# learningOrchestra/learningOrchestra

Measured on NVIDIA H100. Metric: rows/sec project+cast+histogram 100M×32 fp64→fp32; HBM GB/s vs peak @1/2/4/8 GPU, higher is better.
Workload: dtype f64->f32

## Files before the change

### learningorchestra_b200/csrc/kernels.cuh

```cuda
#pragma once
#include <cstdint>
#include <cuda_runtime.h>
#include "parse_number.cuh"
#include "format_number.cuh"

namespace lo {

constexpr int kThreads      = 256;
constexpr int kVec          = 4;
constexpr int kBatch        = 4;
constexpr int kBatches      = 15;
constexpr int kVecPerThread = kBatch * kBatches;
constexpr int kElemsPerThread = kVec * kVecPerThread;
constexpr int kTileRows     = kThreads * kElemsPerThread;
constexpr int kHalf         = kThreads * kVec / 2;
constexpr int kHistRows     = 64;
constexpr int kHistSmemBytes = (kHistRows * kThreads + 256) * 4;

#ifndef LO_PF_BATCH
#define LO_PF_BATCH 5
#endif
#ifndef LO_PF_NBUF
#define LO_PF_NBUF 2
#endif
// ... 295 lines not shown
    __threadfence();
    asm volatile("red.release.gpu.global.add.u64 [%0], %1;" :: "l"(G.gen), "l"(1ull) : "memory");
    asm volatile("st.release.gpu.global.u64 [%0], %1;" :: "l"(G.epi_seq), "l"(G.step + 1ull) : "memory");
}

__device__ __forceinline__ void group_root_epilogue(const GroupStep &G, int n, int first, int stride, bool signal) {
    for (int i = first; i < n; i += stride) {
        const unsigned long long c = ld_relaxed_sys(G.shared + i);
        G.result[i] = c;
        for (int p = 0; p < G.npeers; ++p)
            if (G.peer_result[p]) G.peer_result[p][i] = c;
        G.shared[i] = 0ull;
    }
    if (signal) {
        __syncthreads();
        __threadfence_system();
        if ((int)threadIdx.x < G.npeers) red_release_sys_add(G.peer_clean[threadIdx.x], 1ull);
    }
}

__device__ __forceinline__ void group_wait_generation(const GroupStep &G) {
    if (G.gen_target == 0ull) return;
    if (threadIdx.x == 0) {
        unsigned long long v;
        const unsigned long long t0 = globaltimer_ns();
        for (;;) {
            asm volatile("ld.acquire.gpu.global.u64 %0, [%1];" : "=l"(v) : "l"(G.gen) : "memory");
            if (v >= G.gen_target) break;
            if (globaltimer_ns() - t0 > G.timeout_ns) { atomicAdd(G.timed_out, 1ull); break; }
            __nanosleep(64);
        }
    }
    __syncthreads();
}

__device__ __forceinline__ void group_finish_column(const GroupStep &G, unsigned j, int nb, int k, unsigned tiles_per_col,
                                                    volatile uint32_t *sflag) {
    __syncthreads();
    if (threadIdx.x == 0) {
        __threadfence();
        *sflag = (atomicAdd(G.col_ticket + j, 1u) == tiles_per_col - 1u) ? 1u : 0u;
    }
    __syncthreads();
    if (*sflag == 0u) return;
    __threadfence();
    if (threadIdx.x == 0) {
        G.col_ticket[j] = 0u;
        if (G.clean) wait_flag_ge(G.clean, G.clean_target, G.timeout_ns, G.timed_out);
    }
    __syncthreads();
    for (int b = threadIdx.x; b < nb; b += blockDim.x) {
        unsigned long long *src = G.local + (long long)j * nb + b;
        const unsigned long long c = ld_relaxed_gpu(src);
        if (c) {
            asm volatile("red.relaxed.sys.global.add.u64 [%0], %1;" :: "l"(G.shared + (long long)j * nb + b), "l"(c) : "memory");
            *src = 0ull;
        }
    }
    __syncthreads();
    if (threadIdx.x == 0) {
        __threadfence_system();
        const bool last = atomicAdd(G.done_ticket, 1u) == (unsigned)k - 1u;
        if (last) {
            *G.done_ticket = 0u;
            __threadfence_system();
            red_release_sys_add(G.arrived, 1ull);
            if (!G.is_root) asm volatile("red.release.gpu.global.add.u64 [%0], %1;" :: "l"(G.gen), "l"(1ull) : "memory");
        }
        *sflag = (last && G.is_root) ? 2u : 0u;
        if (*sflag == 2u) {
            epilogue_turn_wait(G);
            if (!wait_flag_ge(G.arrived, G.arrive_target, G.timeout_ns, G.timed_out)) *sflag = 3u;
        }
    }
    __syncthreads();
    if (*sflag == 2u) group_root_epilogue(G, k * nb, threadIdx.x, blockDim.x, true);
    else if (*sflag == 3u && (int)threadIdx.x < G.npeers) red_release_sys_add(G.peer_clean[threadIdx.x], 1ull);
    if (*sflag >= 2u) {
        __syncthreads();
        if (threadIdx.x == 0) epilogue_turn_done(G);
    }
}

template <int OUT, bool HIST, bool ALIGNED, bool EDGES>
__global__ void __launch_bounds__(kThreads, LO_MIN_CTAS)
k_project_cast_hist(const char *__restrict__ in_base, long long in_pitch,
                    char *__restrict__ out_base, long long out_pitch,
                    long long nrows, unsigned tiles_per_col, unsigned long long *__restrict__ counts,
                    const float *__restrict__ edges, const __grid_constant__ ColsF64 P, const __grid_constant__ GroupStep G) {
    extern __shared__ uint32_t smem[];
    if (G.overlap) asm volatile("griddepcontrol.launch_dependents;" ::: "memory");
    const unsigned j    = blockIdx.x / tiles_per_col;
    const unsigned tile = blockIdx.x - j * tiles_per_col;
    const long long r0  = (long long)tile * kTileRows;
    const long long n   = min((long long)kTileRows, nrows - r0);

    const double *in = reinterpret_cast<const double *>(in_base + (long long)P.col[j] * in_pitch) + r0;
    float  *out32 = nullptr;
    double *out64 = nullptr;
    if (OUT == 1) out32 = reinterpret_cast<float *>(out_base + (long long)j * out_pitch) + r0;
    if (OUT == 2) out64 = reinterpret_cast<double *>(out_base + (long long)j * out_pitch) + r0;

    BinParams B = {0.f, 0.f, 1.f, 1.f, 0};
    int rows = 0;
    uint8_t *priv = reinterpret_cast<uint8_t *>(smem) + 4 * threadIdx.x;
    if (HIST) {
        B.lo = P.lo[j]; B.hi = P.hi[j]; B.w = P.w[j];
        B.r = __frcp_rn(B.w);
        B.last = P.nbins - 1;
        rows = (P.nbins + 3) >> 2;
    }
    EdgeParams E = {0.f, 0.f, 0u};
    if (HIST && EDGES) {
        uint4 *tab = reinterpret_cast<uint4 *>(reinterpret_cast<char *>(smem) + kHistSmemBytes);
        load_edge_table(tab, edges + (long long)j * (P.nbins + 1), P.nbins);
        E = edge_params(B.lo, B.w, tab);
    }

    if (ALIGNED && n == kTileRows) {
        double v[kPfBuf][kPfBatch][4];
        const double *src = in + 2 * (long long)threadIdx.x;
#pragma unroll
        for (int pb = 0; pb < kPfBuf - 1; ++pb)
#pragma unroll
            for (int u = 0; u < kPfBatch; ++u)
                ldg_split4_stream(src + (long long)(pb * kPfBatch + u) * kThreads * kVec, kHalf, v[pb][u]);
        if (HIST) zero_private(smem, rows);
        const long long t2 = 2 * (long long)threadIdx.x;
#pragma unroll 1
        for (int b0 = 0; b0 < kPfBatches; b0 += kPfBuf) {
            const double *rsrc = src + (long long)b0 * (kPfBatch * kThreads * kVec);
            float  *rout32 = (OUT == 1) ? out32 + t2 + (long long)b0 * (kPfBatch * kThreads * kVec) : nullptr;
            double *rout64 = (OUT == 2) ? out64 + t2 + (long long)b0 * (kPfBatch * kThreads * kVec) : nullptr;
#pragma unroll
            for (int s = 0; s < kPfBuf; ++s) {
                const int b  = b0 + s;
                const int nb = b + kPfBuf - 1;
                if (nb < kPfBatches) {
#pragma unroll
                    for (int u = 0; u < kPfBatch; ++u)
                        ldg_split4_stream(rsrc + ((s + kPfBuf - 1) * kPfBatch + u) * kThreads * kVec, kHalf,
                                          v[(s + kPfBuf - 1) % kPfBuf][u]);
                }
#pragma unroll
                for (int u = 0; u < kPfBatch; ++u) {
                    const int e = (s * kPfBatch + u) * kThreads * kVec;
                    float f0 = cast_f64_f32(v[s][u][0]), f1 = cast_f64_f32(v[s][u][1]);
                    float f2 = cast_f64_f32(v[s][u][2]), f3 = cast_f64_f32(v[s][u][3]);
                    if (OUT == 1) stg_split4_stream(rout32 + e, kHalf, f0, f1, f2, f3);
                    if (OUT == 2) stg_split4_stream(rout64 + e, kHalf, v[s][u]);
                    if (HIST && EDGES) {
                        bump_edge(priv, f0, E); bump_edge(priv, f1, E); bump_edge(priv, f2, E); bump_edge(priv, f3, E);
                    } else if (HIST) {
                        bump4(priv, bin_index_f32<false>(f0, B), bin_index_f32<false>(f1, B),
                              bin_index_f32<false>(f2, B), bin_index_f32<false>(f3, B));
                    }
                }
            }
        }
    } else if (ALIGNED) {
        if (HIST) zero_private(smem, rows);
#pragma unroll 1
        for (int b = 0; b < kBatches; ++b) {
            const long long e0 = (long long)b * kBatch * kThreads * kVec + 2 * threadIdx.x;
            if (e0 >= n) break;
            double v[kBatch][4];
            if (e0 + (long long)(kBatch - 1) * kThreads * kVec + kHalf + 2 <= n) {
#pragma unroll
                for (int u = 0; u < kBatch; ++u) ldg_split4_stream(in + e0 + (long long)u * kThreads * kVec, kHalf, v[u]);
#pragma unroll
                for (int u = 0; u < kBatch; ++u) {
                    const long long e = e0 + (long long)u * kThreads * kVec;
                    float f0 = cast_f64_f32(v[u][0]), f1 = cast_f64_f32(v[u][1]);
                    float f2 = cast_f64_f32(v[u][2]), f3 = cast_f64_f32(v[u][3]);
                    if (OUT == 1) stg_split4_stream(out32 + e, kHalf, f0, f1, f2, f3);
                    if (OUT == 2) stg_split4_stream(out64 + e, kHalf, v[u]);
                    if (HIST && EDGES) {
                        bump_edge(priv, f0, E); bump_edge(priv, f1, E); bump_edge(priv, f2, E); bump_edge(priv, f3, E);
                    } else if (HIST) {
                        bump4(priv, bin_index_f32<false>(f0, B), bin_index_f32<false>(f1, B),
                              bin_index_f32<false>(f2, B), bin_index_f32<false>(f3, B));
                    }
                }
            } else {
#pragma unroll 1
                for (int u = 0; u < kBatch; ++u) {
                    const long long e = e0 + (long long)u * kThreads * kVec;
#pragma unroll 1
                    for (int q = 0; q < kVec; ++q) {
                        const long long eq = e + (q & 1) + (q >> 1) * kHalf;
                        if (eq < n) {
                            double x = ldg64_stream(in + eq);
                            float  f = cast_f64_f32(x);
                            if (OUT == 1) out32[eq] = f;
                            if (OUT == 2) out64[eq] = x;
                            if (HIST && EDGES) bump_edge(priv, f, E);
                            else if (HIST) bin_f32<false>(priv, f, B);
                        }
                    }
                }
            }
        }
    } else {
        if (HIST) zero_private(smem, rows);
#pragma unroll 1
        for (int i = 0; i < kElemsPerThread; ++i) {
            const long long e = (long long)i * kThreads + threadIdx.x;
            if (e >= n) break;
            double x = ldg64_stream(in + e);
            float  f = cast_f64_f32(x);
            if (OUT == 1) out32[e] = f;
            if (OUT == 2) out64[e] = x;
            if (HIST && EDGES) bump_edge(priv, f, E);
            else if (HIST) bin_f32<false>(priv, f, B);
        }
    }

    if (HIST) {
        if (G.mode == 0) {
            fold_and_flush(smem, rows, P.nbins, counts + (long long)j * P.nbins);
        } else {
            group_wait_generation(G);
            fold_and_flush(smem, rows, P.nbins, G.local + (long long)j * P.nbins);
            group_finish_column(G, j, P.nbins, P.k, tiles_per_col, smem);
        }
    }
}

constexpr int kWBThreads   = 512;
constexpr int kWBSmemWords = 16384;
constexpr int kWBSmemWordsMax = 57344;
constexpr int kWBVecs      = 4;
constexpr int kWBRoundRows = kWBThreads * kVec * kWBVecs;
// ... 705 lines not shown
```

### learningorchestra_b200/csrc/loexec.cu

```cuda
#include "loexec.h"
#include "kernels.cuh"

#include <cub/device/device_scan.cuh>

#include <algorithm>
#include <atomic>
#include <condition_variable>
#include <cctype>
#include <chrono>
#include <cmath>
#include <cstdarg>
#include <cstdio>
#include <cstdlib>
#include <cstring>
#include <memory>
#include <mutex>
#include <new>
#include <string>
#include <type_traits>
#include <utility>
#include <vector>

namespace {

thread_local std::string g_err;

int fail(int code, const char *fmt, ...) {
    char buf[512];
    va_list ap;
    va_start(ap, fmt);
    vsnprintf(buf, sizeof buf, fmt, ap);
    va_end(ap);
    g_err = buf;
    (void)cudaGetLastError();
    return code;
}

#define LO_CUDA(call)                                                                        \
    do {                                                                                     \
        cudaError_t e_ = (call);                                                             \
        if (e_ != cudaSuccess) {                                                             \
            int code_ = (e_ == cudaErrorMemoryAllocation) ? LO_ERR_NOMEM : LO_ERR_CUDA;      \
            return fail(code_, "%s failed: %s (%s:%d)", #call, cudaGetErrorString(e_),       \
                        __FILE__, __LINE__);                                                 \
        }                                                                                    \
    } while (0)

#define LO_TRY(call)                 \
    do {                             \
        int rc_ = (call);            \
        if (rc_ != LO_OK) return rc_; \
    } while (0)

size_t dtype_size(int dtype) {
    switch (dtype) {
        case LO_F64: return 8;
        case LO_F32: return 4;
        case LO_U8:  return 1;
        case LO_U32: return 4;
        default:     return 0;
    }
}

}

struct lo_table {
    int       dtype;
    int64_t   nrows;
    int32_t   ncols;
    int64_t   pitch;
    char     *base;
    bool      owned;
    int       device;
};

constexpr int kSlots = 3;
constexpr int kMaxStageSets = 4;

struct StageSet {
    cudaStream_t compute = nullptr, h2d = nullptr, d2h = nullptr;
    char        *in[kSlots]  = {nullptr, nullptr, nullptr};
    char        *out[kSlots] = {nullptr, nullptr, nullptr};
    size_t       in_bytes = 0, out_bytes = 0;
    unsigned long long *counts = nullptr;
    size_t       counts_n = 0;
    cudaEvent_t  ev_h2d[kSlots] = {}, ev_k[kSlots] = {}, ev_d2h[kSlots] = {};
};

struct EdgeTable {
    int32_t            nbins = 0;
    std::vector<float> lo, hi;
    float             *dev = nullptr;
    size_t             bytes = 0;
    cudaEvent_t        ready = nullptr;
    std::vector<cudaEvent_t> uses;
    uint64_t           last_use = 0;
};
constexpr int kEdgeTables = 8;

struct lo_ctx {
    int          device;
    int          sm_count;
    size_t       hbm_bytes;
    cudaStream_t stream;
    std::atomic<int64_t> launches{0};
    std::atomic<bool> use_tma{false};
    std::mutex   pool_mu;
    std::condition_variable pool_cv;
    std::vector<StageSet *> free_sets;
    int          nsets = 0;
    std::mutex   edge_mu;
    cudaStream_t edge_stream = nullptr;
    std::vector<std::unique_ptr<EdgeTable>> edge_tables;
    uint64_t     edge_tick = 0;
    std::atomic<int64_t> divide_launches{0};
};

namespace {

cudaStream_t pick(lo_ctx *ctx, void *stream) { return stream ? (cudaStream_t)stream : ctx->stream; }

int check_ctx(const lo_ctx *ctx) {
    if (!ctx) return fail(LO_ERR_INVALID, "ctx is NULL");
    cudaError_t e = cudaSetDevice(ctx->device);
    if (e != cudaSuccess) return fail(LO_ERR_CUDA, "cudaSetDevice(%d): %s", ctx->device, cudaGetErrorString(e));
    return LO_OK;
}

cudaError_t launched(lo_ctx *ctx, int n) {
    const cudaError_t e = cudaGetLastError();
    if (e == cudaSuccess) ctx->launches.fetch_add(n, std::memory_order_relaxed);
    return e;
}

bool aligned32(const lo_table *t) {
    return ((uintptr_t)t->base % 32 == 0) && (t->pitch % 32 == 0);
}

int check_cols(const lo_table *in, const int32_t *col_idx, int32_t k) {
    if (k <= 0) return fail(LO_ERR_INVALID, "k must be > 0 (got %d)", k);
    if (!col_idx) return fail(LO_ERR_INVALID, "col_idx is NULL");
    for (int j = 0; j < k; ++j)
        if (col_idx[j] < 0 || col_idx[j] >= in->ncols)
            return fail(LO_ERR_INVALID, "col_idx[%d] = %d outside [0, %d)", j, col_idx[j], in->ncols);
    return LO_OK;
}

int check_spec(const lo_hist_spec *spec, int32_t k, float *w_out ) {
    if (spec->nbins < 1 || spec->nbins > LO_MAX_BINS)
        return fail(LO_ERR_INVALID, "nbins = %d outside [1, %d]", spec->nbins, LO_MAX_BINS);
    if (spec->flags != 0) return fail(LO_ERR_INVALID, "unknown lo_hist_spec.flags 0x%x", spec->flags);
    if (!spec->lo || !spec->hi) return fail(LO_ERR_INVALID, "lo_hist_spec.lo / .hi is NULL");
    for (int j = 0; j < k; ++j) {
        const float lo = spec->lo[j], hi = spec->hi[j];
        volatile float span = hi - lo;
        volatile float w    = span / (float)spec->nbins;
        if (!(std::isfinite(lo) && std::isfinite(hi)) || !(hi > lo) || !std::isfinite(w) || !(w > 0.0f))
            return fail(LO_ERR_INVALID, "histogram range of column %d is not usable: lo=%g hi=%g nbins=%d",
                        j, (double)lo, (double)hi, spec->nbins);
        w_out[j] = w;
    }
    return LO_OK;
}

template <typename K>
int allow_smem(K kernel, int bytes) {
    LO_CUDA(cudaFuncSetAttribute(kernel, cudaFuncAttributeMaxDynamicSharedMemorySize, bytes));
    return LO_OK;
}

template <int OUT>
int allow_smem_hist() {
    LO_TRY(allow_smem(lo::k_project_cast_hist<OUT, true, true, true>, lo::kEdgeSmemBytes));
    LO_TRY(allow_smem(lo::k_project_cast_hist<OUT, true, true, false>, lo::kHistSmemBytes));
    LO_TRY(allow_smem(lo::k_project_cast_hist<OUT, true, false, true>, lo::kEdgeSmemBytes));
    LO_TRY(allow_smem(lo::k_project_cast_hist<OUT, true, false, false>, lo::kHistSmemBytes));
    return LO_OK;
}

bool fastdiv_ok(float w) {
    uint32_t bits;
    memcpy(&bits, &w, 4);
    if ((bits & 0x007FFFFFu) == 0x007FFFFFu) return false;
    return w >= 0x1p-100f && w <= 0x1p100f;
}

bool edges_ok(float w) { return w >= 0x1p-100f && w <= 0x1p100f; }

int bin_ieee_host(float f, float lo, float w, int last) {
// ... 91 lines not shown
        nt->bytes = n * 4;
        std::vector<float> h(n);
        for (int j = 0; j < P.k; ++j) hist_edges(P.lo[j], P.hi[j], P.w[j], P.nbins, h.data() + (size_t)j * (P.nbins + 1));
        cudaError_t e = cudaMallocAsync((void **)&nt->dev, nt->bytes, ctx->edge_stream);
        if (e == cudaSuccess) e = cudaMemcpyAsync(nt->dev, h.data(), nt->bytes, cudaMemcpyHostToDevice, ctx->edge_stream);
        if (e == cudaSuccess) e = cudaEventCreateWithFlags(&nt->ready, cudaEventDisableTiming);
        if (e == cudaSuccess) e = cudaEventRecord(nt->ready, ctx->edge_stream);
        if (e != cudaSuccess) {
            edge_retire(ctx, nt.get());
            return fail(e == cudaErrorMemoryAllocation ? LO_ERR_NOMEM : LO_ERR_CUDA, "edge table upload: %s",
                        cudaGetErrorString(e));
        }
        t = nt.get();
        ctx->edge_tables.push_back(std::move(nt));
    }
    LO_CUDA(cudaStreamWaitEvent(s, t->ready, 0));
    t->last_use = ++ctx->edge_tick;
    *out = t;
    return LO_OK;
}

int edge_used(EdgeTable *t, cudaStream_t s) {
    t->uses.erase(std::remove_if(t->uses.begin(), t->uses.end(), [](cudaEvent_t e) {
                      if (cudaEventQuery(e) != cudaSuccess) return false;
                      cudaEventDestroy(e);
                      return true;
                  }), t->uses.end());
    (void)cudaGetLastError();
    cudaEvent_t e = nullptr;
    LO_CUDA(cudaEventCreateWithFlags(&e, cudaEventDisableTiming));
    const cudaError_t r = cudaEventRecord(e, s);
    if (r != cudaSuccess) {
        cudaEventDestroy(e);
        return fail(LO_ERR_CUDA, "edge table use: %s", cudaGetErrorString(r));
    }
    t->uses.push_back(e);
    return LO_OK;
}

template <typename K>
int allow_smem_tma(K kernel) {
    LO_CUDA(cudaFuncSetAttribute(kernel, cudaFuncAttributeMaxDynamicSharedMemorySize, lo::kTmaSmemBytes));
    return LO_OK;
}

int configure_kernels() {
    LO_TRY(allow_smem_tma(lo::k_project_cast_hist_tma<0, true, true>));
    LO_TRY(allow_smem_tma(lo::k_project_cast_hist_tma<1, true, true>));
    LO_TRY(allow_smem_tma(lo::k_project_cast_hist_tma<2, true, true>));
    LO_TRY(allow_smem_tma(lo::k_project_cast_hist_tma<1, false, false>));
    LO_TRY(allow_smem_tma(lo::k_project_cast_hist_tma<2, false, false>));
    LO_TRY(allow_smem_hist<0>());
    LO_TRY(allow_smem_hist<1>());
    LO_TRY(allow_smem_hist<2>());
    LO_CUDA(cudaFuncSetAttribute(lo::k_hist_u8_cols_lanes<true>, cudaFuncAttributeMaxDynamicSharedMemorySize, lo::kU8LSmemBytes));
    LO_CUDA(cudaFuncSetAttribute(lo::k_hist_u8_cols_lanes<false>, cudaFuncAttributeMaxDynamicSharedMemorySize, lo::kU8LSmemBytes));
    LO_CUDA(cudaFuncSetAttribute(lo::k_project_cast_hist_bins<0, true>, cudaFuncAttributeMaxDynamicSharedMemorySize, lo::kWBSmemWordsMax * 4));
    LO_CUDA(cudaFuncSetAttribute(lo::k_project_cast_hist_bins<1, true>, cudaFuncAttributeMaxDynamicSharedMemorySize, lo::kWBSmemWordsMax * 4));
    LO_CUDA(cudaFuncSetAttribute(lo::k_project_cast_hist_bins<2, true>, cudaFuncAttributeMaxDynamicSharedMemorySize, lo::kWBSmemWordsMax * 4));
    LO_CUDA(cudaFuncSetAttribute(lo::k_project_cast_hist_bins<0, false>, cudaFuncAttributeMaxDynamicSharedMemorySize, lo::kWBSmemWordsMax * 4));
    LO_CUDA(cudaFuncSetAttribute(lo::k_project_cast_hist_bins<1, false>, cudaFuncAttributeMaxDynamicSharedMemorySize, lo::kWBSmemWordsMax * 4));
    LO_CUDA(cudaFuncSetAttribute(lo::k_project_cast_hist_bins<2, false>, cudaFuncAttributeMaxDynamicSharedMemorySize, lo::kWBSmemWordsMax * 4));
    return LO_OK;
}

const lo::GroupStep kNoGroup = {};

template <typename... KArgs, typename... Args>
cudaError_t launch_kernel(void (*kernel)(KArgs...), unsigned grid, unsigned block, size_t smem, cudaStream_t s, bool overlap,
                          Args &&...args) {
    cudaLaunchConfig_t cfg = {};
    cfg.gridDim = dim3(grid);
    cfg.blockDim = dim3(block);
    cfg.dynamicSmemBytes = smem;
    cfg.stream = s;
    cudaLaunchAttribute attr[1];
    attr[0].id = cudaLaunchAttributeProgrammaticStreamSerialization;
    attr[0].val.programmaticStreamSerializationAllowed = 1;
    cfg.attrs = attr;
    cfg.numAttrs = overlap ? 1 : 0;
    return cudaLaunchKernelEx(&cfg, kernel, std::forward<Args>(args)...);
}

template <int OUT, bool HIST>
int launch_f64(lo_ctx *ctx, const lo_table *in, const lo_table *out, int32_t out_col0,
               const lo::ColsF64 &P, unsigned long long *counts, bool aligned, const lo::GroupStep &G, cudaStream_t s) {
    std::unique_lock<std::mutex> edge_lock(ctx->edge_mu, std::defer_lock);
    EdgeTable *et = nullptr;
    if (HIST) {
        edge_lock.lock();
        LO_TRY(edge_acquire(ctx, P, s, &et));
        if (!et) {
            edge_lock.unlock();
            ctx->divide_launches.fetch_add(1, std::memory_order_relaxed);
        }
    }
    const float *edges = et ? et->dev : nullptr;
    const size_t smem = !HIST ? 0 : edges ? lo::kEdgeSmemBytes : lo::kHistSmemBytes;
    char *out_base = out ? out->base + (int64_t)out_col0 * out->pitch : nullptr;
    const long long out_pitch = out ? out->pitch : 0;
    bool fast = HIST;
    for (int j = 0; HIST && j < P.k; ++j) fast = fast && fastdiv_ok(P.w[j]);
    if (ctx->use_tma.load(std::memory_order_relaxed) && aligned && fast == HIST && in->nrows >= lo::kTileRows && G.mode == 0) {
        const unsigned full_tiles = (unsigned)(in->nrows / lo::kTileRows);
        const unsigned long long tblocks = (unsigned long long)full_tiles * (unsigned)P.k;
        if (tblocks > 0x7fffffffull) return fail(LO_ERR_INVALID, "table too large for one launch (%llu tiles)", tblocks);
        lo::k_project_cast_hist_tma<OUT, HIST, HIST><<<(unsigned)tblocks, lo::kThreads + 32, lo::kTmaSmemBytes, s>>>(
            in->base, in->pitch, out_base, out_pitch, in->nrows, full_tiles, counts, P);
        LO_CUDA(launched(ctx, 1));
        const int64_t done = (int64_t)full_tiles * lo::kTileRows;
        if (done == in->nrows) return LO_OK;
        const char *ib = in->base + done * 8;
        char *ob = out ? out->base + done * (int64_t)dtype_size(out->dtype) + (int64_t)out_col0 * out->pitch : nullptr;
        if (edges) lo::k_project_cast_hist<OUT, HIST, true, true><<<(unsigned)P.k, lo::kThreads, smem, s>>>(
                       ib, in->pitch, ob, out_pitch, in->nrows - done, 1u, counts, edges, P, kNoGroup);
        else       lo::k_project_cast_hist<OUT, HIST, true, false><<<(unsigned)P.k, lo::kThreads, smem, s>>>(
                       ib, in->pitch, ob, out_pitch, in->nrows - done, 1u, counts, edges, P, kNoGroup);
        LO_CUDA(launched(ctx, 1));
        if (et) LO_TRY(edge_used(et, s));
        return LO_OK;
    }
    const unsigned tiles_per_col = (unsigned)((in->nrows + lo::kTileRows - 1) / lo::kTileRows);
    const unsigned long long blocks = (unsigned long long)tiles_per_col * (unsigned)P.k;
    if (blocks > 0x7fffffffull) return fail(LO_ERR_INVALID, "table too large for one launch (%llu tiles)", blocks);
    const char *ib = in->base;
    const long long ip = in->pitch, nr = in->nrows;
#define LO_LAUNCH(AL, ED)                                                                                        \
    LO_CUDA(launch_kernel(lo::k_project_cast_hist<OUT, HIST, AL, ED>, (unsigned)blocks, lo::kThreads, smem, s,    \
                          G.overlap != 0, ib, ip, out_base, out_pitch, nr, tiles_per_col, counts, edges, P, G))
    if (aligned) { if (edges) LO_LAUNCH(true, true); else LO_LAUNCH(true, false); }
    else         { if (edges) LO_LAUNCH(false, true); else LO_LAUNCH(false, false); }
#undef LO_LAUNCH
    LO_CUDA(launched(ctx, 1));
    if (et) LO_TRY(edge_used(et, s));
    return LO_OK;
}

template <int OUT>
int launch_f64_bins(lo_ctx *ctx, const lo_table *in, const lo_table *out, int32_t out_col0,
                    const lo::ColsF64 &P, unsigned long long *counts, bool aligned, const lo::GroupStep &G, cudaStream_t s) {
    char *out_base = out ? out->base + (int64_t)out_col0 * out->pitch : nullptr;
    const long long out_pitch = out ? out->pitch : 0;
    bool fast = true;
    for (int j = 0; j < P.k; ++j) fast = fast && fastdiv_ok(P.w[j]);
    int slots_log2 = -1;
    if (P.nbins <= lo::kWBSmemWords) {
        slots_log2 = 0;
        while (slots_log2 < 5 && (P.nbins << (slots_log2 + 1)) <= lo::kWBSmemWords) ++slots_log2;
    } else if (P.nbins <= lo::kWBSmemWordsMax) {
        slots_log2 = 0;
    }
    const size_t smem = slots_log2 >= 0 ? (size_t)(P.nbins << slots_log2) * 4 : 16;
    const int64_t slots = (int64_t)ctx->sm_count * 2;
    int64_t want = (in->nrows * (int64_t)P.k) / (4 * slots);
    want = std::max<int64_t>(lo::kWBRoundRows, std::min<int64_t>(want, (int64_t)1 << 24));
    const int64_t chunk_rows = (want / lo::kWBRoundRows) * lo::kWBRoundRows;
    const unsigned chunks_per_col = (unsigned)((in->nrows + chunk_rows - 1) / chunk_rows);
    const unsigned long long blocks = (unsigned long long)chunks_per_col * (unsigned)P.k;
    if (blocks > 0x7fffffffull) return fail(LO_ERR_INVALID, "table too large for one launch (%llu chunks)", blocks);
    const char *ib = in->base;
    const long long ip = in->pitch, nr = in->nrows;
    if (fast) LO_CUDA(launch_kernel(lo::k_project_cast_hist_bins<OUT, true>, (unsigned)blocks, (unsigned)lo::kWBThreads, smem, s, G.overlap != 0,
                                    ib, ip, out_base, out_pitch, nr, chunks_per_col, (long long)chunk_rows, slots_log2, (int)aligned, counts, P, G));
    else      LO_CUDA(launch_kernel(lo::k_project_cast_hist_bins<OUT, false>, (unsigned)blocks, (unsigned)lo::kWBThreads, smem, s, G.overlap != 0,
                                    ib, ip, out_base, out_pitch, nr, chunks_per_col, (long long)chunk_rows, slots_log2, (int)aligned, counts, P, G));
    LO_CUDA(launched(ctx, 1));
    return LO_OK;
}

int project_cast_hist_impl(lo_ctx *ctx, const lo_table *in, const int32_t *col_idx, int32_t k,
                           lo_table *out, const lo_hist_spec *spec, uint64_t *counts_dev, cudaStream_t s,
                           const lo::GroupStep *group = nullptr) {
    if (!in) return fail(LO_ERR_INVALID, "input table is NULL");
    if (in->dtype != LO_F64) return fail(LO_ERR_INVALID, "input table must be LO_F64 (got dtype %d)", in->dtype);
    LO_TRY(check_cols(in, col_idx, k));
    int out_mode = 0;
    if (out) {
        if (out->dtype == LO_F32) out_mode = 1;
        else if (out->dtype == LO_F64) out_mode = 2;
        else return fail(LO_ERR_INVALID, "output table must be LO_F32 or LO_F64 (got dtype %d)", out->dtype);
        if (out->nrows != in->nrows) return fail(LO_ERR_INVALID, "output rows %lld != input rows %lld",
                                                  (long long)out->nrows, (long long)in->nrows);
        if (out->ncols < k) return fail(LO_ERR_INVALID, "output has %d columns, need %d", out->ncols, k);
        if (out->device != in->device) return fail(LO_ERR_INVALID, "tables live on different devices");
    }
    if (!out && !spec) return fail(LO_ERR_INVALID, "nothing to do: no output table and no histogram spec");
    std::vector<float> w;
    if (spec) {
        if (!counts_dev) return fail(LO_ERR_INVALID, "counts_dev is NULL");
        w.resize(k);
        LO_TRY(check_spec(spec, k, w.data()));
    }
    if (group && (!spec || k > lo::kMaxColsF64))
        return fail(LO_ERR_INVALID, "a group step needs a histogram spec and k <= %d (got %d)", lo::kMaxColsF64, k);
    if (in->nrows == 0 && !group) return LO_OK;
    const bool aligned = aligned32(in) && (!out || aligned32(out));
    const lo::GroupStep &G = group ? *group : kNoGroup;

    for (int32_t c0 = 0; c0 < k; c0 += lo::kMaxColsF64) {
        lo::ColsF64 P;
        P.k     = std::min<int32_t>(lo::kMaxColsF64, k - c0);
        P.nbins = spec ? spec->nbins : 0;
        for (int j = 0; j < P.k; ++j) {
            P.col[j] = col_idx[c0 + j];
            P.lo[j]  = spec ? spec->lo[c0 + j] : 0.f;
            P.hi[j]  = spec ? spec->hi[c0 + j] : 0.f;
            P.w[j]   = spec ? w[c0 + j] : 1.f;
        }
        unsigned long long *cnt = spec ? (unsigned long long *)counts_dev + (int64_t)c0 * spec->nbins : nullptr;
        int rc;
        if (spec && spec->nbins > LO_TILE_BINS) {
            if (out_mode == 0)      rc = launch_f64_bins<0>(ctx, in, out, c0, P, cnt, aligned, G, s);
// ... 220 lines not shown
        for (void *p : v) cudaFreeAsync(p, s);
        v.clear();
    }
    int finish(lo_host_timing *timing) {
        release(scratch);
        latch(cudaStreamSynchronize(s));
        if (!ok()) {
            release(kept);
            return fail(rc, "%s", msg.c_str());
        }
        if (timing) {
            double kernel_ms = 0;
            for (size_t i = 0; i + 1 < marks.size(); i += 2) {
                float t = 0.f;
                if (cudaEventElapsedTime(&t, marks[i], marks[i + 1]) == cudaSuccess) kernel_ms += t;
            }
            timing->total_ms  = std::chrono::duration<double, std::milli>(std::chrono::steady_clock::now() - t0).count();
            timing->h2d_bytes = h2d;
            timing->d2h_bytes = d2h;
            timing->launches  = ctx->launches.load() - launches0;
            timing->kernel_ms = kernel_ms;
        }
        return LO_OK;
    }
};

}

extern "C" {

int lo_abi_version(void) { return LO_ABI_VERSION; }

const char *lo_last_error(void) { return g_err.c_str(); }

int lo_device_count(int *out) {
    if (!out) return fail(LO_ERR_INVALID, "out is NULL");
    int n = 0;
    cudaError_t e = cudaGetDeviceCount(&n);
    if (e != cudaSuccess) {
        *out = 0;
        return fail(LO_ERR_NO_DEVICE, "cudaGetDeviceCount: %s", cudaGetErrorString(e));
    }
    *out = n;
    return LO_OK;
}

int lo_init(int device, lo_ctx **out) {
    if (!out) return fail(LO_ERR_INVALID, "out is NULL");
    *out = nullptr;
    int n = 0;
    cudaError_t e = cudaGetDeviceCount(&n);
    if (e != cudaSuccess || n == 0)
        return fail(LO_ERR_NO_DEVICE, "no CUDA device (%s); libloexec has no CPU fallback",
                    e != cudaSuccess ? cudaGetErrorString(e) : "device count 0");
    if (device < 0 || device >= n) return fail(LO_ERR_INVALID, "device %d outside [0, %d)", device, n);
    cudaDeviceProp prop;
    LO_CUDA(cudaGetDeviceProperties(&prop, device));
    if (prop.major != 9 || prop.minor != 0)
        return fail(LO_ERR_NO_DEVICE, "device %d is sm_%d%d; libloexec is built for sm_90a only", device,
                    prop.major, prop.minor);
    int reserved = 0;
    LO_CUDA(cudaDeviceGetAttribute(&reserved, cudaDevAttrReservedSharedMemoryPerBlock, device));
    if (reserved != LO_SMEM_WINDOW_BASE)
        return fail(LO_ERR_NO_DEVICE, "device %d reserves %d bytes of shared memory per block, the kernels assume %d",
                    device, reserved, LO_SMEM_WINDOW_BASE);
    LO_CUDA(cudaSetDevice(device));
    lo_ctx *ctx = new (std::nothrow) lo_ctx;
    if (!ctx) return fail(LO_ERR_NOMEM, "out of host memory");
    ctx->device    = device;
    ctx->sm_count  = prop.multiProcessorCount;
    ctx->hbm_bytes = prop.totalGlobalMem;
    ctx->stream = nullptr;
    auto setup = [&]() -> int {
        LO_CUDA(cudaStreamCreateWithFlags(&ctx->stream, cudaStreamNonBlocking));
        LO_CUDA(cudaStreamCreateWithFlags(&ctx->edge_stream, cudaStreamNonBlocking));
        cudaMemPool_t pool = nullptr;
        LO_CUDA(cudaDeviceGetDefaultMemPool(&pool, device));
        uint64_t keep = 8ull << 30;
        if (const char *e = getenv("LOEXEC_POOL_KEEP_MB")) keep = (uint64_t)std::max<long long>(0, atoll(e)) << 20;
        LO_CUDA(cudaMemPoolSetAttribute(pool, cudaMemPoolAttrReleaseThreshold, &keep));
        return configure_kernels();
    };
    if (const char *e = getenv("LOEXEC_TMA")) ctx->use_tma.store(e[0] == '1');
    const int rc = setup();
    if (rc != LO_OK) {
        const std::string msg = g_err;
        lo_shutdown(ctx);
        g_err = msg;
        return rc;
    }
    *out = ctx;
    return LO_OK;
}

int lo_shutdown(lo_ctx *ctx) {
    if (!ctx) return LO_OK;
    cudaSetDevice(ctx->device);
    cudaDeviceSynchronize();
    for (StageSet *st : ctx->free_sets) stage_set_destroy(st);
    ctx->free_sets.clear();
    if (ctx->edge_stream) {
        for (const auto &t : ctx->edge_tables) edge_retire(ctx, t.get());
        cudaStreamSynchronize(ctx->edge_stream);
        cudaStreamDestroy(ctx->edge_stream);
    }
    ctx->edge_tables.clear();
    if (ctx->stream) cudaStreamDestroy(ctx->stream);
    delete ctx;
    return LO_OK;
}

int lo_ctx_device(const lo_ctx *ctx, int *device, int *sm_count, size_t *hbm_bytes) {
    if (!ctx) return fail(LO_ERR_INVALID, "ctx is NULL");
    if (device) *device = ctx->device;
    if (sm_count) *sm_count = ctx->sm_count;
    if (hbm_bytes) *hbm_bytes = ctx->hbm_bytes;
    return LO_OK;
}

int lo_sync(lo_ctx *ctx, void *stream) {
    LO_TRY(check_ctx(ctx));
    LO_CUDA(cudaStreamSynchronize(pick(ctx, stream)));
    return LO_OK;
}

int lo_set_tma(lo_ctx *ctx, int enabled) {
    if (!ctx) return fail(LO_ERR_INVALID, "ctx is NULL");
    ctx->use_tma.store(enabled != 0, std::memory_order_relaxed);
    return LO_OK;
}

int lo_launch_count(const lo_ctx *ctx, int64_t *out) {
    if (!ctx || !out) return fail(LO_ERR_INVALID, "NULL argument");
    *out = ctx->launches.load(std::memory_order_relaxed);
    return LO_OK;
}

int lo_host_alloc(lo_ctx *ctx, size_t bytes, void **out) {
    LO_TRY(check_ctx(ctx));
    if (!out) return fail(LO_ERR_INVALID, "out is NULL");
    *out = nullptr;
    if (bytes == 0) return LO_OK;
    LO_CUDA(cudaHostAlloc(out, bytes, cudaHostAllocPortable));
    return LO_OK;
}

int lo_host_alloc_flags(lo_ctx *ctx, size_t bytes, int32_t flags, void **out) {
    LO_TRY(check_ctx(ctx));
    if (!out) return fail(LO_ERR_INVALID, "out is NULL");
    if (flags & ~LO_HOST_WRITE_COMBINED) return fail(LO_ERR_INVALID, "unknown flags 0x%x", flags);
    *out = nullptr;
    if (bytes == 0) return LO_OK;
    LO_CUDA(cudaHostAlloc(out, bytes, cudaHostAllocPortable | ((flags & LO_HOST_WRITE_COMBINED) ? cudaHostAllocWriteCombined : 0)));
    return LO_OK;
}

int lo_host_free(lo_ctx *ctx, void *p) {
    LO_TRY(check_ctx(ctx));
    if (p) LO_CUDA(cudaFreeHost(p));
    return LO_OK;
}

int lo_table_alloc(lo_ctx *ctx, int dtype, int64_t nrows, int32_t ncols, lo_table **out) {
    LO_TRY(check_ctx(ctx));
    if (!out) return fail(LO_ERR_INVALID, "out is NULL");
    *out = nullptr;
// ... 644 lines not shown
```

Measured before the change: 7.871 billion.

## Interleave full-tile batches across concurrently resident CTAs for DRAM locality

```diff
diff --git a/learningorchestra_b200/csrc/kernels.cuh b/learningorchestra_b200/csrc/kernels.cuh
--- a/learningorchestra_b200/csrc/kernels.cuh
+++ b/learningorchestra_b200/csrc/kernels.cuh
@@ -401,11 +401,19 @@
     }
 }
 
+constexpr int kPfBatchRows = kPfBatch * kThreads * kVec;
+
+template <typename T>
+__device__ __forceinline__ T *opaque(T *p) {
+    asm("" : "+l"(p));
+    return p;
+}
+
 template <int OUT, bool HIST, bool ALIGNED, bool EDGES>
 __global__ void __launch_bounds__(kThreads, LO_MIN_CTAS)
 k_project_cast_hist(const char *__restrict__ in_base, long long in_pitch,
                     char *__restrict__ out_base, long long out_pitch,
-                    long long nrows, unsigned tiles_per_col, unsigned long long *__restrict__ counts,
+                    long long nrows, unsigned tiles_per_col, unsigned tile_group, unsigned long long *__restrict__ counts,
                     const float *__restrict__ edges, const __grid_constant__ ColsF64 P, const __grid_constant__ GroupStep G) {
     extern __shared__ uint32_t smem[];
     if (G.overlap) asm volatile("griddepcontrol.launch_dependents;" ::: "memory");
@@ -414,7 +422,8 @@
     const long long r0  = (long long)tile * kTileRows;
     const long long n   = min((long long)kTileRows, nrows - r0);
 
-    const double *in = reinterpret_cast<const double *>(in_base + (long long)P.col[j] * in_pitch) + r0;
+    const double *col_in = reinterpret_cast<const double *>(in_base + (long long)P.col[j] * in_pitch);
+    const double *in = col_in + r0;
     float  *out32 = nullptr;
     double *out64 = nullptr;
     if (OUT == 1) out32 = reinterpret_cast<float *>(out_base + (long long)j * out_pitch) + r0;
@@ -422,7 +431,9 @@
 
     BinParams B = {0.f, 0.f, 1.f, 1.f, 0};
     int rows = 0;
-    uint8_t *priv = reinterpret_cast<uint8_t *>(smem) + 4 * threadIdx.x;
+    unsigned tid = threadIdx.x;
+    asm("" : "+r"(tid));
+    uint8_t *priv = reinterpret_cast<uint8_t *>(smem) + 4 * tid;
     if (HIST) {
         B.lo = P.lo[j]; B.hi = P.hi[j]; B.w = P.w[j];
         B.r = __frcp_rn(B.w);
@@ -437,37 +448,42 @@
     }
 
     if (ALIGNED && n == kTileRows) {
+        const unsigned full  = (unsigned)(nrows / kTileRows);
+        const unsigned t     = tile % tile_group;
+        const unsigned first = tile - t;
+        const unsigned bstride = min(tile_group, full - first) * (unsigned)kPfBatchRows;
+        const long long row0 = (long long)first * kTileRows + (long long)t * kPfBatchRows + 2 * (long long)threadIdx.x;
+        const double *src = opaque(col_in + row0);
+        float  *dst32 = (OUT == 1) ? opaque(reinterpret_cast<float *>(out_base + (long long)j * out_pitch) + row0) : nullptr;
+        double *dst64 = (OUT == 2) ? opaque(reinterpret_cast<double *>(out_base + (long long)j * out_pitch) + row0) : nullptr;
         double v[kPfBuf][kPfBatch][4];
-        const double *src = in + 2 * (long long)threadIdx.x;
 #pragma unroll
         for (int pb = 0; pb < kPfBuf - 1; ++pb)
 #pragma unroll
             for (int u = 0; u < kPfBatch; ++u)
-                ldg_split4_stream(src + (long long)(pb * kPfBatch + u) * kThreads * kVec, kHalf, v[pb][u]);
+                ldg_split4_stream(src + pb * bstride + u * kThreads * kVec, kHalf, v[pb][u]);
         if (HIST) zero_private(smem, rows);
-        const long long t2 = 2 * (long long)threadIdx.x;
+        unsigned off = 0;
 #pragma unroll 1
-        for (int b0 = 0; b0 < kPfBatches; b0 += kPfBuf) {
-            const double *rsrc = src + (long long)b0 * (kPfBatch * kThreads * kVec);
-            float  *rout32 = (OUT == 1) ? out32 + t2 + (long long)b0 * (kPfBatch * kThreads * kVec) : nullptr;
-            double *rout64 = (OUT == 2) ? out64 + t2 + (long long)b0 * (kPfBatch * kThreads * kVec) : nullptr;
+        for (int b0 = 0; b0 < kPfBatches; b0 += kPfBuf, off += kPfBuf * bstride) {
 #pragma unroll
             for (int s = 0; s < kPfBuf; ++s) {
                 const int b  = b0 + s;
                 const int nb = b + kPfBuf - 1;
                 if (nb < kPfBatches) {
+                    const double *p = src + (off + (s + kPfBuf - 1) * bstride);
 #pragma unroll
                     for (int u = 0; u < kPfBatch; ++u)
-                        ldg_split4_stream(rsrc + ((s + kPfBuf - 1) * kPfBatch + u) * kThreads * kVec, kHalf,
-                                          v[(s + kPfBuf - 1) % kPfBuf][u]);
+                        ldg_split4_stream(p + u * kThreads * kVec, kHalf, v[(s + kPfBuf - 1) % kPfBuf][u]);
                 }
+                const unsigned boff = off + s * bstride;
 #pragma unroll
                 for (int u = 0; u < kPfBatch; ++u) {
-                    const int e = (s * kPfBatch + u) * kThreads * kVec;
+                    const int e = u * kThreads * kVec;
                     float f0 = cast_f64_f32(v[s][u][0]), f1 = cast_f64_f32(v[s][u][1]);
                     float f2 = cast_f64_f32(v[s][u][2]), f3 = cast_f64_f32(v[s][u][3]);
-                    if (OUT == 1) stg_split4_stream(rout32 + e, kHalf, f0, f1, f2, f3);
-                    if (OUT == 2) stg_split4_stream(rout64 + e, kHalf, v[s][u]);
+                    if (OUT == 1) stg_split4_stream(dst32 + boff + e, kHalf, f0, f1, f2, f3);
+                    if (OUT == 2) stg_split4_stream(dst64 + boff + e, kHalf, v[s][u]);
                     if (HIST && EDGES) {
                         bump_edge(priv, f0, E); bump_edge(priv, f1, E); bump_edge(priv, f2, E); bump_edge(priv, f3, E);
                     } else if (HIST) {
diff --git a/learningorchestra_b200/csrc/loexec.cu b/learningorchestra_b200/csrc/loexec.cu
--- a/learningorchestra_b200/csrc/loexec.cu
+++ b/learningorchestra_b200/csrc/loexec.cu
@@ -105,6 +105,9 @@
     cudaStream_t stream;
     std::atomic<int64_t> launches{0};
     std::atomic<bool> use_tma{false};
+    unsigned     tile_group_fixed = 0;
+    std::mutex   tile_mu;
+    std::vector<std::pair<const void *, unsigned>> tile_groups;
     std::mutex   pool_mu;
     std::condition_variable pool_cv;
     std::vector<StageSet *> free_sets;
@@ -362,6 +365,20 @@
     return cudaLaunchKernelEx(&cfg, kernel, std::forward<Args>(args)...);
 }
 
+constexpr unsigned kMaxTileGroup = 65536;
+template <typename K>
+int tile_group(lo_ctx *ctx, K kernel, size_t smem, unsigned *out) {
+    if (ctx->tile_group_fixed) { *out = std::min(ctx->tile_group_fixed, kMaxTileGroup); return LO_OK; }
+    std::lock_guard<std::mutex> lock(ctx->tile_mu);
+    for (const auto &c : ctx->tile_groups)
+        if (c.first == (const void *)kernel) { *out = c.second; return LO_OK; }
+    int per_sm = 0;
+    LO_CUDA(cudaOccupancyMaxActiveBlocksPerMultiprocessor(&per_sm, kernel, lo::kThreads, smem));
+    *out = std::min((unsigned)std::max(1, per_sm * ctx->sm_count), kMaxTileGroup);
+    ctx->tile_groups.emplace_back((const void *)kernel, *out);
+    return LO_OK;
+}
+
 template <int OUT, bool HIST>
 int launch_f64(lo_ctx *ctx, const lo_table *in, const lo_table *out, int32_t out_col0,
                const lo::ColsF64 &P, unsigned long long *counts, bool aligned, const lo::GroupStep &G, cudaStream_t s) {
@@ -393,9 +410,9 @@
         const char *ib = in->base + done * 8;
         char *ob = out ? out->base + done * (int64_t)dtype_size(out->dtype) + (int64_t)out_col0 * out->pitch : nullptr;
         if (edges) lo::k_project_cast_hist<OUT, HIST, true, true><<<(unsigned)P.k, lo::kThreads, smem, s>>>(
-                       ib, in->pitch, ob, out_pitch, in->nrows - done, 1u, counts, edges, P, kNoGroup);
+                       ib, in->pitch, ob, out_pitch, in->nrows - done, 1u, 1u, counts, edges, P, kNoGroup);
         else       lo::k_project_cast_hist<OUT, HIST, true, false><<<(unsigned)P.k, lo::kThreads, smem, s>>>(
-                       ib, in->pitch, ob, out_pitch, in->nrows - done, 1u, counts, edges, P, kNoGroup);
+                       ib, in->pitch, ob, out_pitch, in->nrows - done, 1u, 1u, counts, edges, P, kNoGroup);
         LO_CUDA(launched(ctx, 1));
         if (et) LO_TRY(edge_used(et, s));
         return LO_OK;
@@ -405,9 +422,12 @@
     if (blocks > 0x7fffffffull) return fail(LO_ERR_INVALID, "table too large for one launch (%llu tiles)", blocks);
     const char *ib = in->base;
     const long long ip = in->pitch, nr = in->nrows;
-#define LO_LAUNCH(AL, ED)                                                                                        \
+    unsigned tg = 1;
+#define LO_LAUNCH(AL, ED) do {                                                                                   \
+    LO_TRY(tile_group(ctx, lo::k_project_cast_hist<OUT, HIST, AL, ED>, smem, &tg));                              \
     LO_CUDA(launch_kernel(lo::k_project_cast_hist<OUT, HIST, AL, ED>, (unsigned)blocks, lo::kThreads, smem, s,    \
-                          G.overlap != 0, ib, ip, out_base, out_pitch, nr, tiles_per_col, counts, edges, P, G))
+                          G.overlap != 0, ib, ip, out_base, out_pitch, nr, tiles_per_col, tg, counts, edges, P, G)); \
+    } while (0)
     if (aligned) { if (edges) LO_LAUNCH(true, true); else LO_LAUNCH(true, false); }
     else         { if (edges) LO_LAUNCH(false, true); else LO_LAUNCH(false, false); }
 #undef LO_LAUNCH
@@ -794,6 +814,10 @@
         return configure_kernels();
     };
     if (const char *e = getenv("LOEXEC_TMA")) ctx->use_tma.store(e[0] == '1');
+    if (const char *e = getenv("LOEXEC_TILE_ORDER")) {
+        if (!strcmp(e, "contiguous")) ctx->tile_group_fixed = 1;
+        else if (atoi(e) > 0) ctx->tile_group_fixed = (unsigned)atoi(e);
+    }
     const int rc = setup();
     if (rc != LO_OK) {
         const std::string msg = g_err;
```

After: 7.918 billion (median of 6 runs). No clear change (+0.6%).
